# LSquarzoni/SNN_Event-based_Optical_Flow

Hardware: AMD Instinct MI355X
Metric: events/sec (train step) LIFFireNet T=10 128x128 (higher is better)
Workload: dtype fp32; 1 GPU; LIFFireNet train step: T=10 x 1000-event windows, 128x128, batch 8/GPU, base_num_channels 8, EventWarping + Adam; global_batch=8, parallelism=dp1, hip_graph=True, launch_order=wavefront

## Files before the change

include/snnflow.h:

```cpp
#ifndef SNNFLOW_H
#define SNNFLOW_H

#include <stdint.h>

#ifdef __cplusplus
extern "C" {
#endif

#define SNNFLOW_ABI_VERSION 41

#define SNNFLOW_E_ARG (-1)
#define SNNFLOW_E_CHANNELS (-2)

#define SNNFLOW_TILE_H 8
#define SNNFLOW_TILE_W 32

typedef struct snnflow_neuron {
    const float* bn_weight;
    const float* bn_bias;
    float* running_mean;
    float* running_var;
    int64_t* num_batches_tracked;
    const float* beta;
    const float* threshold;
// ... 101 lines not shown
    const uint16_t* wd_ff; const uint16_t* wd_rec;
    float* wslab_ff; float* wslab_rec; const float* s_prev; int wslab_accumulate;
    const float* x; int64_t xs_b, xs_c, xs_h, xs_w;
} snnflow_layer_bwd_args;
int snnflow_layer_bwd(const snnflow_layer_bwd_args* a, void* stream);

#define SNNFLOW_MAX_SLOT_TASKS 4
int snnflow_fwd_slot(const snnflow_conv_fwd_args* conv, int nconv, const snnflow_lif_fwd_args* lif,
                     void* stream);
int snnflow_bwd_slot(const snnflow_layer_bwd_args* layer, int nlayer, const snnflow_lif_bwd_args* lif,
                     void* stream);
int snnflow_slot_supported(int c, int cin0);
#define SNNFLOW_MAX_CHAIN_TASKS 7
int snnflow_bwd_chain(const snnflow_layer_bwd_args* layer, int nlayer, const unsigned char* pair,
                      const snnflow_lif_bwd_args* lif, void* stream);
int snnflow_set_pipe(int fwd_tiles_per_block, int bwd_tiles_per_block);
int snnflow_get_pipe(int which);

#define SNNFLOW_MAX_LAYERS 8

typedef struct snnflow_wgrad_step {
    const float* g_cur;
    const float* y;
    const float* x; int64_t xs_b, xs_c, xs_h, xs_w;
    const float* s_prev;
    const float* stats;
    const float* bnc;
    const uint8_t* x_bits; const uint8_t* s_prev_bits;
} snnflow_wgrad_step;
#define SNNFLOW_MAX_WGRAD_STEPS 32
// ... 516 lines not shown
```

snn_event-based_optical_flow_amd/csrc/lif_layers.hip:

```cpp
#include <cmath>
#include <string>
#include <type_traits>

#include "snnflow_dev.h"
#include "snnflow_tile.h"

#ifndef SNNFLOW_PROBE
#define SNNFLOW_PROBE 0
#endif
#define PROBE_OFF(bit) ((SNNFLOW_PROBE & (bit)) != 0)

#ifndef SNNFLOW_SP32
#define SNNFLOW_SP32 2
#endif
#ifndef SNNFLOW_LATE_D_REC8
#define SNNFLOW_LATE_D_REC8 1
#endif
#ifndef SNNFLOW_LATE_D_FF8
#define SNNFLOW_LATE_D_FF8 1
#endif
#ifndef SNNFLOW_EARLY_G_REC8
#define SNNFLOW_EARLY_G_REC8 1
#endif
#ifndef SNNFLOW_L32_WAVES
// ... 2915 lines not shown
        const float m = beta[c] * mem[i] + x[i];
        const bool s = m >= thr[c];
        spk[i] = s ? 1.0f : 0.0f;
        mout[i] = s ? 0.0f : m;
    }
}

constexpr int kSlotTasks = SNNFLOW_MAX_SLOT_TASKS;

enum SlotKind : int {
    SK_HEAD1, SK_HEAD2, SK_HEAD4, SK_HEAD5,
    SK_PLAIN, SK_PLAIN_REC,
    SK_LIF, SK_LIF_REC,
    SK_TOP, SK_TOP_PRED,
    SK_LIF_P, SK_LIF_REC_P,
    SK_CHAIN
};

struct FwdSlotParams {
    snnflow_conv_fwd_args conv[kSlotTasks];
    snnflow_lif_fwd_args lif;
    int kind[kSlotTasks], blk0[kSlotTasks], nblk[kSlotTasks];
    int ntask;
};
constexpr int kBwdTasks = SNNFLOW_MAX_CHAIN_TASKS, kBwdNodes = kBwdTasks + 1;
struct ByteRange { int off, len; };
constexpr int kNrnA0 = offsetof(snnflow_neuron, running_mean), kNrnA1 = offsetof(snnflow_neuron, beta);
constexpr int kNrnB0 = offsetof(snnflow_neuron, momentum), kNrnB1 = offsetof(snnflow_neuron, bn_train);
constexpr int kBwdOffN = offsetof(snnflow_layer_bwd_args, n), kBwdOffP = offsetof(snnflow_layer_bwd_args, prev);
constexpr int kBwdKeepN = 5;
constexpr ByteRange kBwdKeep[kBwdKeepN] = {
    {0, kBwdOffN + kNrnA0},
    {kBwdOffN + kNrnA1, kNrnB0 - kNrnA1},
    {kBwdOffN + kNrnB1, kBwdOffP + kNrnA0 - (kBwdOffN + kNrnB1)},
    {kBwdOffP + kNrnA1, kNrnB0 - kNrnA1},
    {kBwdOffP + kNrnB1, (int)sizeof(snnflow_layer_bwd_args) - (kBwdOffP + kNrnB1)}};
constexpr int bwd_keep_bytes(int n) { return n == 0 ? 0 : bwd_keep_bytes(n - 1) + kBwdKeep[n - 1].len; }
constexpr bool bwd_keep_aligned(int n) {
    return n == 0 || (kBwdKeep[n - 1].off % 8 == 0 && kBwdKeep[n - 1].len % 8 == 0 && kBwdKeep[n - 1].len > 0 && bwd_keep_aligned(n - 1));
// ... 19 lines not shown
constexpr int cmax(int a, int b) { return a > b ? a : b; }

template <int C>
constexpr bool kSlotAllKinds = C == 8;

constexpr int kFragC8 = 3 * 3 * 256;
constexpr int kPipeRaw = 2 * HN * 16, kPipeSpk = HN * 8 * 2, kPipeFrag = kFragC8 * 2;
template <bool REC>
struct PipeFwdLds {
    static constexpr int RAWY = 0, RAWM = kPipeRaw, SPK = 2 * kPipeRaw, RSPK = SPK + kPipeSpk;
    static constexpr int FF = RSPK + (REC ? kPipeSpk : 0), FR = FF + kPipeFrag;
    static constexpr int BYTES = FR + (REC ? kPipeFrag : 0);
    static constexpr int FLOATS = BYTES / 4;
};

template <int C>
struct SlotLds {
    static constexpr int FWD_ALL = cmax(cmax(ConvFwdLds<1, C, false, false, 2>::FLOATS, ConvFwdLds<5, C, false, false, 2>::FLOATS),
                                        cmax(ConvFwdLds<C, C, false, false, 2>::FLOATS, ConvFwdLds<C, C, false, true, 2>::FLOATS));
    static constexpr int FWD_P = C == 8 ? PipeFwdLds<true>::FLOATS : 0;
    static constexpr int FWD = cmax(cmax(cmax(kSlotAllKinds<C> ? FWD_ALL : 0, kLifQFwdLds<C>), FWD_P),
                                    cmax(cmax(ConvFwdLds<2, C, false, false, 2>::FLOATS, ConvFwdLds<4, C, false, false, 2>::FLOATS),
                                         cmax(ConvFwdLds<C, C, true, false, 2>::FLOATS, ConvFwdLds<C, C, true, true, 2>::FLOATS)));
    static constexpr bool BFG = C >= 16;
    static constexpr int BWD_ALL = cmax(LayerBwdLds<C, C, false, false, 2>::FLOATS, LayerBwdLds<C, C, false, true, 2>::FLOATS);
    static constexpr int BWD = cmax(cmax(cmax(kSlotAllKinds<C> ? BWD_ALL : 0, kLifQBwdLds<C, true>),
                                         cmax(LayerBwdLds<2, C, false, false, 2>::FLOATS, LayerBwdLds<4, C, false, false, 2>::FLOATS)),
                                    cmax(LayerBwdLds<C, C, true, false, 2, BFG>::FLOATS,
                                         LayerBwdLds<C, C, true, true, 2, BFG>::FLOATS));
};

template <typename T>
__device__ inline T kernarg_copy(const __attribute__((address_space(4))) T* p) {
    static_assert(sizeof(T) % 4 == 0, "dword-sized struct");
    T r;
// ... 347 lines not shown
        if ((lane & 15) == 0) {
#pragma unroll
            for (int j = 0; j < 8; ++j) red[wv][lane >> 4][j] = v[j];
        }
        __syncthreads();
        if (tid < 2 * C) {
            const int c = tid & 7, sq = tid >> 3, qd = c >> 2, j = sq * 4 + (c & 3);
            double s = 0.0;
#pragma unroll
            for (int w = 0; w < 8; ++w) s += (double)red[w][qd][j] + (double)red[w][qd + 2][j];
            atomicAdd(acc_shard(a.acc, 2 * C, g.bid) + sq * C + c, s);
        }
    }
}

template <int C>
__global__ __launch_bounds__(NT * 2, C == 8 ? 6 : 1) void k_fwd_slot(FwdSlotParams) {
    typedef const __attribute__((address_space(4))) FwdSlotParams* cptr;
    const cptr pp = (cptr)__builtin_amdgcn_kernarg_segment_ptr();
    Grid g;
    const int k = slot_task(pp, g);
    if (g.bid >= g.nb) return;
    __shared__ __attribute__((aligned(16))) float pool[SlotLds<C>::FWD];
    switch (pp->kind[k]) {
#define FWD_CONV(ALL, KIND, ...)                              \
    case KIND: {                                              \
        if constexpr (ALL || kSlotAllKinds<C>) {              \
            const snnflow_conv_fwd_args a = task_args(&pp->conv[k]);         \
            conv_fwd_body<__VA_ARGS__>(a, g, pool);           \
        }                                                     \
        break;                                                \
    }
        FWD_CONV(false, SK_HEAD1, 1, C, false, false, 2)
        FWD_CONV(true, SK_HEAD2, 2, C, false, false, 2)
        FWD_CONV(true, SK_HEAD4, 4, C, false, false, 2)
        FWD_CONV(false, SK_HEAD5, 5, C, false, false, 2)
        FWD_CONV(false, SK_PLAIN, C, C, false, false, 2)
        FWD_CONV(false, SK_PLAIN_REC, C, C, false, true, 2)
        FWD_CONV(true, SK_LIF, C, C, true, false, 2)
        FWD_CONV(true, SK_LIF_REC, C, C, true, true, 2)
#undef FWD_CONV
        case SK_LIF_P:
        case SK_LIF_REC_P: {
            if constexpr (C == 8) {
                {
                    const snnflow_conv_fwd_args a = task_args(&pp->conv[k]);
                    if (pp->kind[k] == SK_LIF_REC_P) fwd_lif8_pipe<true>(a, g, pool);
                    else fwd_lif8_pipe<false>(a, g, pool);
                }
            }
            break;
        }
        case SK_TOP: {
            if constexpr (kSlotAllKinds<C>) {
                const snnflow_lif_fwd_args a = task_args(&pp->lif);
                lif_fwd_body<C, false, NT * 2>(a, g);
            }
            break;
        }
        case SK_TOP_PRED: {
            const snnflow_lif_fwd_args a = task_args(&pp->lif);
            if constexpr (C >= 16) lif_fwd_q_body<C, true, NT * 2>(a, g, pool);
            else lif_fwd_body<C, true, NT * 2>(a, g);
            break;
// ... 575 lines not shown
        case 4: return layer_bwd_c<4>(*a, s);
        case 8: return layer_bwd_c<8>(*a, s);
        case 16: return layer_bwd_c<16>(*a, s);
        case 32: return layer_bwd_c<32>(*a, s);
        default: SNN_FAIL(SNNFLOW_E_CHANNELS, "layer_bwd: c must be 4, 8, 16 or 32");
    }
}

static bool slot_c(int c) { return c == 8 || c == 16 || c == 32; }

#ifndef SNNFLOW_SLOT_ORDER
#define SNNFLOW_SLOT_ORDER 1
#endif
static int slot_rank(int kind) {
    switch (kind) {
        case SK_LIF_REC_P: case SK_LIF_P: return 0;
        case SK_LIF_REC: case SK_PLAIN_REC: return 0;
        case SK_LIF: case SK_PLAIN: return 1;
        default: return 2;
    }
}

#ifndef SNNFLOW_SLOT_ORDER8
#define SNNFLOW_SLOT_ORDER8 0
#endif
extern "C++" template <typename A>
static void slot_sort(A* args, int* kind, int* nblk, int n, bool reverse = false) {
    if (!SNNFLOW_SLOT_ORDER) return;
    const int sg = reverse ? -1 : 1;
    for (int i = 1; i < n; ++i)
        for (int j = i; j > 0 && sg * slot_rank(kind[j]) < sg * slot_rank(kind[j - 1]); --j) {
// ... 23 lines not shown
    return (nb + 7) / 8 * 8;
}
static bool pipe_fits(int B, int H, int W, int c) { return (int64_t)B * H * W * c * 4 < ((int64_t)1 << 31); }

int snnflow_slot_supported(int c, int cin0) { return slot_c(c) && (cin0 == 2 || cin0 == 4) ? 1 : 0; }

static int slot_ranges(const int* nblk, int n, int* blk0) {
    int b = 0;
    for (int i = 0; i < n; ++i) {
        blk0[i] = b;
        b += (nblk[i] + 7) / 8 * 8;
    }
    return b;
}

int snnflow_fwd_slot(const snnflow_conv_fwd_args* conv, int nconv, const snnflow_lif_fwd_args* lif, void* stream) {
    const int nt = nconv + (lif ? 1 : 0);
    if (nconv < 0 || nt <= 0 || nt > kSlotTasks || (nconv && !conv)) SNN_FAIL(SNNFLOW_E_ARG, "fwd_slot: task count");
    FwdSlotParams p = {};
    const int c = nconv ? conv[0].c : lif->c;
    const int B = nconv ? conv[0].B : lif->B, H = nconv ? conv[0].H : lif->H, W = nconv ? conv[0].W : lif->W;
    if (!slot_c(c)) SNN_FAIL(SNNFLOW_E_CHANNELS, "fwd_slot: c must be 8, 16 or 32");
    for (int i = 0; i < nconv; ++i) {
        const snnflow_conv_fwd_args& a = conv[i];
        if (const int e = conv_fwd_check(&a)) return e;
        if (a.c != c || a.B != B || a.H != H || a.W != W) SNN_FAIL(SNNFLOW_E_ARG, "fwd_slot: tasks of different shapes");
        int kind;
        if (a.lif_in) {
            if (a.cin != c) SNN_FAIL(SNNFLOW_E_CHANNELS, "fwd_slot: lif_in requires cin == c");
            kind = a.wt_rec ? SK_LIF_REC : SK_LIF;
        } else if (a.wt_rec) {
            if (a.cin != c) SNN_FAIL(SNNFLOW_E_CHANNELS, "fwd_slot: recurrent cell requires cin == c");
            kind = SK_PLAIN_REC;
        } else if (a.cin == c) {
            kind = SK_PLAIN;
        } else if (a.cin == 1 || a.cin == 2 || a.cin == 4 || a.cin == 5) {
            kind = a.cin == 1 ? SK_HEAD1 : a.cin == 2 ? SK_HEAD2 : a.cin == 4 ? SK_HEAD4 : SK_HEAD5;
        } else {
            SNN_FAIL(SNNFLOW_E_CHANNELS, "fwd_slot: unsupported cin");
        }
        if (c != 8 && !(kind == SK_HEAD2 || kind == SK_HEAD4 || kind == SK_LIF || kind == SK_LIF_REC))
            SNN_FAIL(SNNFLOW_E_CHANNELS, "fwd_slot: c = 16 / 32 runs the LIFFireNet task kinds only");
        p.conv[i] = a;
        p.nblk[i] = snnflow_conv_blocks(B, H, W);
        if (c == 8 && g_pipe_fwd > 0 && (kind == SK_LIF || kind == SK_LIF_REC) && pipe_fits(B, H, W, c) &&
            !a.prev_spk_bits && !a.s_prev_bits)
            kind = kind == SK_LIF ? SK_LIF_P : SK_LIF_REC_P;
        p.kind[i] = kind;
    }
    const int tpb = g_pipe_fwd;
    for (int i = 0; i < nconv; ++i) {
        if (p.kind[i] != SK_LIF_P && p.kind[i] != SK_LIF_REC_P) continue;
        const int nt = p.nblk[i];
        p.nblk[i] = pipe_blocks(nt, tpb);
        if (p.nblk[i] > (nt + 7) / 8 * 8) p.nblk[i] = (nt + 7) / 8 * 8;
    }
    if (lif) {
        if (const int e = lif_fwd_check(lif)) return e;
        if (lif->c != c || lif->B != B || lif->H != H || lif->W != W)
            SNN_FAIL(SNNFLOW_E_ARG, "fwd_slot: tasks of different shapes");
        if (c != 8 && !lif->pred_w) SNN_FAIL(SNNFLOW_E_CHANNELS, "fwd_slot: c = 16 / 32 top task needs the prediction");
        p.lif = *lif;
        p.kind[nconv] = lif->pred_w ? SK_TOP_PRED : SK_TOP;
        p.nblk[nconv] = slot_top_blocks(c, B, H, W);
    }
    if (c != 8) slot_sort(p.conv, p.kind, p.nblk, nconv);
    else if (SNNFLOW_SLOT_ORDER8) slot_sort(p.conv, p.kind, p.nblk, nconv, SNNFLOW_SLOT_ORDER8 == 2);
    else if (g_pipe_fwd > 0 && g_pipe_order) slot_sort(p.conv, p.kind, p.nblk, nconv, g_pipe_order == 2);
    p.ntask = nt;
    const int nb = slot_ranges(p.nblk, nt, p.blk0);
    const hipStream_t s = (hipStream_t)stream;
    if (c == 8) hipLaunchKernelGGL(k_fwd_slot<8>, dim3(nb), dim3(2 * NT), 0, s, p);
    else if (c == 16) hipLaunchKernelGGL(k_fwd_slot<16>, dim3(nb), dim3(2 * NT), 0, s, p);
    else hipLaunchKernelGGL(k_fwd_slot<32>, dim3(nb), dim3(2 * NT), 0, s, p);
    SNN_CHECK_LAUNCH();
    return 0;
}

int snnflow_eval_slot(const snnflow_eval_fwd_args* tasks, int n, void* stream) {
    if (!tasks || n <= 0 || n > kEvalTasks) SNN_FAIL(SNNFLOW_E_ARG, "eval_slot: task count");
    EvalSlotParams p = {};
    const int B = tasks[0].B, H = tasks[0].H, W = tasks[0].W;
    for (int i = 0; i < n; ++i) {
        const snnflow_eval_fwd_args& a = tasks[i];
        if (a.c != 8) SNN_FAIL(SNNFLOW_E_CHANNELS, "eval_slot: c must be 8");
        if (a.B != B || a.H != H || a.W != W || B <= 0 || H <= 0 || W <= 0)
            SNN_FAIL(SNNFLOW_E_ARG, "eval_slot: tasks of different or empty shapes");
        if (a.n.bn_train) SNN_FAIL(SNNFLOW_E_ARG, "eval_slot: BatchNorm in train mode needs batch statistics (snnflow_fwd_slot)");
        if (!a.state || !a.wt_ff || !a.n.bn_weight || !a.n.bn_bias || !a.n.running_mean || !a.n.running_var ||
            !a.n.beta || !a.n.threshold)
            SNN_FAIL(SNNFLOW_E_ARG, "eval_slot: missing state, weights or neuron parameters");
// ... 337 lines not shown
```

snn_event-based_optical_flow_amd/csrc/snnflow_tile.h:

```cpp
#pragma once

#include <type_traits>

#include "snnflow_dev.h"

#ifndef SNNFLOW_PIN_PF
#define SNNFLOW_PIN_PF 1
#endif

namespace snnflow {


template <int CIN, int NTH = NT>
__device__ void stage_strided(const float* __restrict__ x, int64_t sb, int64_t sc, int64_t sh, int64_t sw,
                              const Tile& tl, int H, int W, float* tile) {
    constexpr int P = Pad<CIN>::v;
    const int tid = threadIdx.x;
    const float* xb = x + (int64_t)tl.b * sb;
    if (sc == 1) {
        for (int e = tid; e < HN * CIN; e += NTH) {
            const int p = e / CIN, ci = e - p * CIN;
            const int r = p / HWD, cc = p - r * HWD;
            const int h = tl.h0 + r - 1, w = tl.w0 + cc - 1;
            tile[p * P + ci] = in_image(h, w, H, W) ? xb[h * sh + w * sw + ci] : 0.0f;
// ... 642 lines not shown
#pragma unroll
                for (int r = 0; r < 4; ++r) out[(row * TW + c0 + g * 4 + r) * PO + n] = v[r];
            }
        }
    }
}

template <int N>
__device__ inline void pin(float (&v)[N]) {
#pragma unroll
    for (int i = 0; i < N; ++i) asm volatile("" : "+v"(v[i]));
}

constexpr int kSumScratch = 8 * 4 * 48;
__device__ inline float* sum_scratch() {
    __shared__ float buf[kSumScratch];
    return buf;
}

template <int NV, int PARTS, typename Dst>
__device__ void block_atomic_sum_parts(const float (&v)[NV], Dst dst) {
    constexpr int WPP = NT / 64, NW = WPP * PARTS;
    if constexpr (NW * 4 * NV > kSumScratch) {
        __shared__ float wred[NW][NV];
        const int lane = threadIdx.x & 63, wv = threadIdx.x >> 6;
#pragma unroll
        for (int j = 0; j < NV; ++j) {
            const float s = wave_total(v[j]);
            if (lane == 0) wred[wv][j] = s;
        }
        __syncthreads();
// ... 165 lines not shown
```

snn_event-based_optical_flow_amd/snnflow/_lib.py:

```python
import ctypes
import os

import torch

_HERE = os.path.dirname(os.path.abspath(__file__))
LIB_PATH = os.environ.get("SNNFLOW_LIB", os.path.join(_HERE, "libsnnflow.so"))

P = ctypes.c_void_p
I32 = ctypes.c_int
I64 = ctypes.c_int64
F32 = ctypes.c_float
F64 = ctypes.c_double

TILE_H, TILE_W = 8, 32
ABI_VERSION = 41
THETA_SCRATCH = 1024 * 32


class Neuron(ctypes.Structure):
    _fields_ = [("bn_weight", P), ("bn_bias", P), ("running_mean", P), ("running_var", P),
                ("num_batches_tracked", P), ("beta", P), ("threshold", P),
                ("momentum", F64), ("eps", F64), ("bn_train", I32), ("zero_reset", I32)]


# ... 330 lines not shown
    "snnflow_iwe_scratch_floats": (I64, [I32, I32, I32, I32, I32, I32]),
    "snnflow_iwe_acc_doubles": (I32, [I32, I32, I32, I32]),
    "snnflow_iwe_corners": (I32, [P, P, I32, I32, F32, I32, I32, F32, I32, P, P, P]),
    "snnflow_iwe_interpolate": (I32, [P, P, P, I64, I32, I32, I32, I32, P, P]),
    "snnflow_iwe_corners_bwd": (I32, [P, P, I32, I32, F32, I32, I32, F32, P, P, P]),
    "snnflow_iwe_interpolate_bwd": (I32, [P, P, I64, I32, I32, I32, I32, P, P, P]),
    "snnflow_lif_export": (I32, [P, P, P, P, I32, I32, I32, P, P, P]),
    "snnflow_lif_theta_subtract": (I32, [P, P, P, I64, I32, P, P, P]),
    "snnflow_clip_grad_norm": (I32, [P, I64, F32, F32, P, P]),
    "snnflow_clip_grad_norm_large": (I32, [P, I64, F32, F32, P, P, P]),
    "snnflow_clip_adam": (I32, [P, P]),
    "snnflow_eval_slot": (I32, [P, I32, P]),
    "snnflow_count_nonzero": (I32, [P, P, I32, P, P]),
    "snnflow_fwd_slot": (I32, [ctypes.POINTER(ConvFwdArgs), I32, ctypes.POINTER(LifFwdArgs), P]),
    "snnflow_bwd_slot": (I32, [ctypes.POINTER(LayerBwdArgs), I32, ctypes.POINTER(LifBwdArgs), P]),
    "snnflow_bwd_chain": (I32, [ctypes.POINTER(LayerBwdArgs), I32, ctypes.POINTER(ctypes.c_ubyte),
                                ctypes.POINTER(LifBwdArgs), P]),
    "snnflow_slot_supported": (I32, [I32, I32]),
    "snnflow_set_pipe": (I32, [I32, I32]),
    "snnflow_get_pipe": (I32, [I32]),
    "snnflow_frag_halfs": (I32, [I32, I32]),
    "snnflow_unet_conv": (I32, [ctypes.POINTER(UNetConvArgs), P]),
    "snnflow_unet_conv_ksplit": (I32, [ctypes.POINTER(UNetConvArgs)]),
    "snnflow_unet_prep_weights": (I32, [P, I32, I32, I32, P, I32, I32, I32, I32, I32, I32, I32, P, P]),
    "snnflow_unet_wgrad": (I32, [ctypes.POINTER(UNetWgradArgs), P]),
    "snnflow_unet_wgrad_partial_floats": (I64, [ctypes.POINTER(UNetWgradArgs)]),
    "snnflow_unet_wgrad_finalize": (I32, [P, I32, P, I32, I32, I32, I32, I32, I32, P, P]),
    "snnflow_unet_lif_bwd": (I32, [ctypes.POINTER(UNetLifBwdArgs), P]),
    "snnflow_unet_lif_bwd_partial_doubles": (I32, [I32, I32, I32]),
    "snnflow_unet_cell_param_grads": (I32, [P, P, P, I32, I32, P, P, P]),
# ... 151 lines not shown
```

snn_event-based_optical_flow_amd/snnflow/engine.py:

```python
import ctypes
import operator
import os

import torch

from . import _lib
from ._lib import check, lib, ptr



def nhwc_state_strides(B, C, H, W):
    return (B * H * W * C, H * W * C, 1, W * C, C)


def empty_state(B, C, H, W, device):
    return torch.empty_strided((2, B, C, H, W), nhwc_state_strides(B, C, H, W), device=device, dtype=torch.float32)


def as_nhwc_state(s):
    two, B, C, H, W = s.shape
    if s.stride() == nhwc_state_strides(B, C, H, W) and s.dtype == torch.float32:
        return s
    out = empty_state(B, C, H, W, s.device)
    out.copy_(s)
# ... 127 lines not shown
        self.L = len(self.cells)
        self.C = self.cells[0].hidden_size
        self.ws = None
        self.prep = PreppedWeights()
        self.bwd_open = False
        self.flat = None
        self.flat_views = None
        self.pending = []
        self.pending_layers = []
        self.slab_live = [False] * self.L
        self.fuse_wgrad = self.C == 8
        fh = os.environ.get("SNNFLOW_FUSE_HEAD")
        self.fuse_head = (self.C >= 16) if fh is None else fh != "0"
        bc = os.environ.get("SNNFLOW_BWD_CHAIN")
        self.bwd_chain = True if bc is None else bc != "0"
        self.spk_bits = os.environ.get("SNNFLOW_SPK_BITS", "1") != "0"
        self.defer_backward = os.environ.get("SNNFLOW_DEFER_BWD", "1") != "0"
        self.keep_seq_states = False
        self.capture_states = False
        self.final_state_out = None
        self.seq_states = None
        self.prep_stale = True
        self.lifs = [c.lif for c in self.cells]
        self.bns = [getattr(c, "batch_norm", c.bn) for c in self.cells]
        self._plist = None
        self._neurons = None
        self._gen = 0

    def __deepcopy__(self, memo):
        import copy
# ... 863 lines not shown
        s = 1 + max((slot[d] for d in deps(n)), default=-1)
        nl = sum(1 for k, _ in n if k < L)
        while s < len(fill) and fill[s] + nl > max_tasks:
            s += 1
        while len(launches) <= s:
            launches.append([])
            fill.append(0)
        slot[n] = s
        fill[s] += nl
        launches[s].append(n)
    for la in launches:
        la.sort(key=lambda n: -n[0][0])
    return launches


def _state_rows(st_all, fin, T):
    rows = [st_all[t] for t in range(st_all.shape[0])]
    return rows + [fin] if fin is not None else rows


class FireNetSequence(torch.autograd.Function):

    @staticmethod
    def forward(ctx, eng, T, *rest):
        L, C = eng.L, eng.C
        xs = list(rest[:T])
        prev = list(rest[T:T + L])
        B, cin0, H, W = xs[0].shape
        dev = xs[0].device
        for x in xs:
# ... 49 lines not shown
        mem_in = [mem0] + [[states[t - 1][l][0] for l in range(L)] for t in range(1, T)]
        s_prev = [sprev0] + [[states[t - 1][l][1] if eng.rec[l] else None for l in range(L)] for t in range(1, T)]
        neurons = eng.neurons()
        train = [bn.training or not bn.track_running_stats for bn in eng.bns]

        fuse = bool(eng.fuse_wgrad)

        bits_on = eng.spk_bits and C in (16, 32) and not fuse
        need_bits = [bits_on and l < L - 1 for l in range(L)]
        bits = (torch.empty(T, L, B * H * W * C // 8, dtype=torch.uint8, device=dev) if any(need_bits)
                else None)
        bptr = [[bits[t, l].data_ptr() if need_bits[l] else None for l in range(L)] for t in range(T)]

        def spk_skip(l, t):
            return t < T - 1 and not eng.keep_seq_states and ((fuse and not eng.rec[l]) or need_bits[l])
        for tasks in wavefront_slots(T, L + 1):
            convs, top = [], None
            for k, t in tasks:
                if k < L:
                    a = _fwd_conv_args(eng, k, B, H, W, cin0, xs[t], ys[t], stats[t], states[t], mem_in[t],
                                       s_prev[t], facc[t], neurons, train, wfwd, wbwd)
                    if k >= 1 and spk_skip(k - 1, t):
                        a.state_spk_skip = 1
                    if k >= 1 and need_bits[k - 1]:
                        a.prev_spk_bits = bptr[t][k - 1]
                    if eng.rec[k] and t >= 1 and need_bits[k]:
                        a.s_prev_bits, a.s_prev = bptr[t - 1][k], None
                    convs.append(a)
                else:
                    top = _fwd_top_args(eng, B, H, W, ys[t], stats[t], states[t], mem_in[t], facc[t], neurons,
                                        flows[t])
                    if spk_skip(L - 1, t):
                        top.state_spk_skip = 1
            arr = (_lib.ConvFwdArgs * max(len(convs), 1))(*convs)
            _lib.call("fwd_slot", lib.snnflow_fwd_slot, arr, len(convs), ctypes.byref(top) if top is not None else None,
                      s)
        _lib.timer_close()

        if eng.capture_states:
            eng.seq_debug = (ys, stats, facc)
        for l in range(L):
            cells[l].lif.mem = states[T - 1][l][0].detach()
        eng.seq_states = [[st.detach() for st in sts] for sts in states] if eng.keep_seq_states else None

        ctx.eng = eng
        ctx.T = T
        ctx.fuse = fuse
        ctx.bptr = bptr
        ctx.bits = bits
        ctx.root = root
        ctx.ext = ext
# ... 246 lines not shown
```

Measured before the change: 68.46 million events/s.

## Chain recurrent layer and following feed-forward layer in one forward pipelined task

Adds a forward chained task (SK_FCHAIN) that fuses a recurrent layer at step t with the next feed-forward layer at step t-1 inside one block. The recurrent layer's spikes are handed over in LDS instead of being reloaded, and the tile loads for the two halves are interleaved. The Python scheduler builds a new wavefront that groups these pairs, which should cut the number of forward launches and the global traffic. In exchange the argument struct and LDS footprint grow, and the dependency graph becomes more intricate.

```diff
diff --git a/include/snnflow.h b/include/snnflow.h
--- a/include/snnflow.h
+++ b/include/snnflow.h
@@ -139,6 +139,8 @@
 #define SNNFLOW_MAX_CHAIN_TASKS 7
 int snnflow_bwd_chain(const snnflow_layer_bwd_args* layer, int nlayer, const unsigned char* pair,
                       const snnflow_lif_bwd_args* lif, void* stream);
+int snnflow_fwd_chain(const snnflow_conv_fwd_args* conv, int nconv, const unsigned char* pair,
+                      const snnflow_lif_fwd_args* lif, void* stream);
 int snnflow_set_pipe(int fwd_tiles_per_block, int bwd_tiles_per_block);
 int snnflow_get_pipe(int which);
 
diff --git a/snn_event-based_optical_flow_amd/csrc/lif_layers.hip b/snn_event-based_optical_flow_amd/csrc/lif_layers.hip
--- a/snn_event-based_optical_flow_amd/csrc/lif_layers.hip
+++ b/snn_event-based_optical_flow_amd/csrc/lif_layers.hip
@@ -2953,15 +2953,18 @@
     SK_LIF, SK_LIF_REC,
     SK_TOP, SK_TOP_PRED,
     SK_LIF_P, SK_LIF_REC_P,
-    SK_CHAIN
+    SK_CHAIN,
+    SK_FCHAIN
 };
 
+constexpr int kFwdTasks = SNNFLOW_MAX_CHAIN_TASKS, kFwdNodes = kFwdTasks + 1;
 struct FwdSlotParams {
-    snnflow_conv_fwd_args conv[kSlotTasks];
+    snnflow_conv_fwd_args conv[kFwdTasks];
     snnflow_lif_fwd_args lif;
-    int kind[kSlotTasks], blk0[kSlotTasks], nblk[kSlotTasks];
+    int kind[kFwdNodes], blk0[kFwdNodes], nblk[kFwdNodes], second[kFwdNodes];
     int ntask;
 };
+static_assert(sizeof(FwdSlotParams) + 256 <= 4096, "kernel arguments: 4 KB with the hidden ones");
 constexpr int kBwdTasks = SNNFLOW_MAX_CHAIN_TASKS, kBwdNodes = kBwdTasks + 1;
 struct ByteRange { int off, len; };
 constexpr int kNrnA0 = offsetof(snnflow_neuron, running_mean), kNrnA1 = offsetof(snnflow_neuron, beta);
@@ -3011,11 +3014,12 @@
     static constexpr int FLOATS = BYTES / 4;
 };
 
+constexpr int kChainFwdFloats = (2 * kPipeRaw + 2 * kPipeSpk + 2 * kPipeFrag) / 4;
 template <int C>
 struct SlotLds {
     static constexpr int FWD_ALL = cmax(cmax(ConvFwdLds<1, C, false, false, 2>::FLOATS, ConvFwdLds<5, C, false, false, 2>::FLOATS),
                                         cmax(ConvFwdLds<C, C, false, false, 2>::FLOATS, ConvFwdLds<C, C, false, true, 2>::FLOATS));
-    static constexpr int FWD_P = C == 8 ? PipeFwdLds<true>::FLOATS : 0;
+    static constexpr int FWD_P = C == 8 ? cmax(PipeFwdLds<true>::FLOATS, kChainFwdFloats) : 0;
     static constexpr int FWD = cmax(cmax(cmax(kSlotAllKinds<C> ? FWD_ALL : 0, kLifQFwdLds<C>), FWD_P),
                                     cmax(cmax(ConvFwdLds<2, C, false, false, 2>::FLOATS, ConvFwdLds<4, C, false, false, 2>::FLOATS),
                                          cmax(ConvFwdLds<C, C, true, false, 2>::FLOATS, ConvFwdLds<C, C, true, true, 2>::FLOATS)));
@@ -3393,12 +3397,257 @@
     }
 }
 
+struct ChainFwdLds {
+    static constexpr int RAWY = 0, RAWM = kPipeRaw, SPK = 2 * kPipeRaw, RSPK = SPK + kPipeSpk;
+    static constexpr int FA = RSPK + kPipeSpk, FB = FA + kPipeFrag;
+    static constexpr int BYTES = FB + kPipeFrag;
+    static constexpr int FLOATS = BYTES / 4;
+    static constexpr int X_FR = 0, X_COEF = kPipeFrag, X_SUMS = X_COEF + 2 * 8 * 16, X_BYTES = X_SUMS + 16 * 8;
+};
+static_assert(ChainFwdLds::BYTES + kPipeFrag == 46464 && ChainFwdLds::FLOATS == kChainFwdFloats, "chained forward pair: LDS budget");
+static_assert(ChainFwdLds::X_BYTES <= kSumScratch * 4 && sizeof(LifCoef) == 16 && ChainFwdLds::X_SUMS % 8 == 0,
+              "chained forward pair: fragments, coefficients and sums in the block-sum scratch");
+
+__device__ inline void chain_issue(const __amdgpu_buffer_rsrc_t rs_y, const __amdgpu_buffer_rsrc_t rs_m, bool has_mem,
+                                   char* lds, const Tile& t, int H, int W, int wv, int lane) {
+    constexpr int C = 8;
+    using L = ChainFwdLds;
+    const int base = ((t.b * H + t.h0 - 1) * W + (t.w0 - 1)) * (C * 4);
+#pragma unroll
+    for (int j = 0; j < 3; ++j) {
+        const int k = wv + 8 * j;
+        if (k >= 22) break;
+        const bool mem = k >= 11;
+        if (mem && !has_mem) continue;
+        const int kk = mem ? k - 11 : k, ee = kk * 64 + lane, p = ee >> 1, r = p / HWD, cc = p - r * HWD;
+        const bool ok = in_image(t.h0 + r - 1, t.w0 + cc - 1, H, W);
+        const uint32_t off = ok ? (uint32_t)(base + (r * W + cc) * (C * 4) + (ee & 1) * 16) : 0x80000000u;
+        if (ee < 2 * HN)
+            __builtin_amdgcn_raw_ptr_buffer_load_lds(mem ? rs_m : rs_y, (lds_void*)(lds + (mem ? L::RAWM : L::RAWY) + kk * 1024),
+                                                     16, off, 0, 0, 0);
+    }
+}
+
+struct ChainHalf {
+    __amdgpu_buffer_rsrc_t rs_y, rs_m;
+    float4* st4;
+    float* y;
+    bool has_mem, zr, spk_skip;
+};
+
+__device__ inline void chain_lif(const ChainHalf& a, int B, int H, int W, const LifCoef* coef, const char* lds, __bf16* spk,
+                                 const Tile& tl, int tid) {
+    constexpr int C = 8, NTB = 2 * NT, R = Halo4<C, NTB>::R;
+    using L = ChainFwdLds;
+    const int qt = tid & 1;
+    const bool has_mem = a.has_mem, zr = a.zr, spk_skip = a.spk_skip;
+    const int64_t plane4 = (int64_t)B * H * W * 2;
+    float4* st4 = a.st4;
+    const LifCoef kc[4] = {coef[4 * qt], coef[4 * qt + 1], coef[4 * qt + 2], coef[4 * qt + 3]};
+#pragma unroll
+    for (int i = 0; i < R; ++i) {
+        const int e = tid + i * NTB;
+        if (e < 2 * HN) {
+            const int p = e >> 1, r = p / HWD, cc = p - r * HWD;
+            const int h = tl.h0 + r - 1, w = tl.w0 + cc - 1;
+            const float4 yv = *reinterpret_cast<const float4*>(lds + L::RAWY + e * 16);
+            const float4 mv = has_mem ? *reinterpret_cast<const float4*>(lds + L::RAWM + e * 16) : make_float4(0.f, 0.f, 0.f, 0.f);
+            float4 sv = make_float4(0.f, 0.f, 0.f, 0.f);
+            if (in_image(h, w, H, W)) {
+                const Lif4 o = zr ? lif_step4(yv, mv, kc, true) : lif_step4(yv, mv, kc, false);
+                sv = o.s;
+                if (r >= 1 && r <= TH && cc >= 1 && cc <= TW) {
+                    const int64_t q = (((int64_t)tl.b * H + h) * W + w) * 2 + qt;
+                    st_state4(st4, q, o.mout);
+                    if (!spk_skip) st_state4(st4, plane4 + q, o.s);
+                }
+            }
+            typedef __bf16 bf16x4 __attribute__((ext_vector_type(4)));
+            *reinterpret_cast<bf16x4*>(spk + p * 8 + 4 * qt) = bf16x4{(__bf16)sv.x, (__bf16)sv.y, (__bf16)sv.z, (__bf16)sv.w};
+        }
+    }
+}
+
+__device__ inline f32x4 chain_conv(bool rec, const char* ff, const char* fr, const __bf16* spk, const __bf16* rspk, int wv,
+                                   int lane) {
+    const int jj = lane & 15, gg = lane >> 4;
+    const bf16x8* fff = reinterpret_cast<const bf16x8*>(ff) + gg * 8 + (jj & 7);
+    const bf16x8* ffr = reinterpret_cast<const bf16x8*>(fr) + gg * 8 + (jj & 7);
+    f32x4 af[2] = {{0.f, 0.f, 0.f, 0.f}, {0.f, 0.f, 0.f, 0.f}}, ar[2] = {{0.f, 0.f, 0.f, 0.f}, {0.f, 0.f, 0.f, 0.f}};
+#pragma unroll
+    for (int ch = 0; ch < 3; ++ch) {
+        const int tap = 4 * ch + gg, ky = tap / 3, kx = tap - 3 * ky;
+        const bf16x8 fh = fff[ch * 96], fm = fff[ch * 96 + 32], fl = fff[ch * 96 + 64];
+#pragma unroll
+        for (int mt = 0; mt < 2; ++mt) {
+            const int off = ((wv + ky) * HWD + mt * 16 + jj + kx) * 8;
+            bf16x8 b = {};
+            if (tap < 9) b = *reinterpret_cast<const bf16x8*>(spk + off);
+            af[mt] = __builtin_amdgcn_mfma_f32_16x16x32_bf16(fl, b, af[mt], 0, 0, 0);
+            af[mt] = __builtin_amdgcn_mfma_f32_16x16x32_bf16(fm, b, af[mt], 0, 0, 0);
+            af[mt] = __builtin_amdgcn_mfma_f32_16x16x32_bf16(fh, b, af[mt], 0, 0, 0);
+        }
+        if (rec) {
+            const bf16x8 rh = ffr[ch * 96], rm = ffr[ch * 96 + 32], rl = ffr[ch * 96 + 64];
+#pragma unroll
+            for (int mt = 0; mt < 2; ++mt) {
+                const int off = ((wv + ky) * HWD + mt * 16 + jj + kx) * 8;
+                bf16x8 b = {};
+                if (tap < 9) b = *reinterpret_cast<const bf16x8*>(rspk + off);
+                ar[mt] = __builtin_amdgcn_mfma_f32_16x16x32_bf16(rl, b, ar[mt], 0, 0, 0);
+                ar[mt] = __builtin_amdgcn_mfma_f32_16x16x32_bf16(rm, b, ar[mt], 0, 0, 0);
+                ar[mt] = __builtin_amdgcn_mfma_f32_16x16x32_bf16(rh, b, ar[mt], 0, 0, 0);
+            }
+        }
+    }
+    f32x4 yv;
+#pragma unroll
+    for (int r = 0; r < 4; ++r) {
+        const float y0 = rec ? af[0][r] + ar[0][r] : af[0][r];
+        const float y1 = rec ? af[1][r] + ar[1][r] : af[1][r];
+        const auto sw = __builtin_amdgcn_permlane32_swap(__builtin_bit_cast(unsigned, y0), __builtin_bit_cast(unsigned, y1),
+                                                         false, false);
+        yv[r] = __builtin_bit_cast(float, sw[0]);
+    }
+    return yv;
+}
+
+__device__ inline void chain_batch_sums(double* acc, const Grid& g, const float (&bs)[4], const float (&bq)[4]) {
+    constexpr int C = 8;
+    const int tid = threadIdx.x, lane = tid & 63, wv = tid >> 6;
+    float v[8] = {bs[0], bs[1], bs[2], bs[3], bq[0], bq[1], bq[2], bq[3]};
+#pragma unroll
+    for (int j = 0; j < 8; ++j) v[j] += dppf<0xB1>(v[j]);
+#pragma unroll
+    for (int j = 0; j < 8; ++j) v[j] += dppf<0x4E>(v[j]);
+#pragma unroll
+    for (int j = 0; j < 8; ++j) v[j] += dppf<0x141>(v[j]);
+#pragma unroll
+    for (int j = 0; j < 8; ++j) v[j] += dppf<0x140>(v[j]);
+    float(*red)[4][8] = reinterpret_cast<float(*)[4][8]>(sum_scratch());
+    if ((lane & 15) == 0) {
+#pragma unroll
+        for (int j = 0; j < 8; ++j) red[wv][lane >> 4][j] = v[j];
+    }
+    __syncthreads();
+    if (acc && tid < 2 * C) {
+        const int c = tid & 7, sq = tid >> 3, qd = c >> 2, j = sq * 4 + (c & 3);
+        double s = 0.0;
+#pragma unroll
+        for (int w = 0; w < 8; ++w) s += (double)red[w][qd][j] + (double)red[w][qd + 2][j];
+        atomicAdd(acc_shard(acc, 2 * C, g.bid) + sq * C + c, s);
+    }
+}
+
+typedef const __attribute__((address_space(4))) snnflow_conv_fwd_args* conv_karg;
+__device__ void fwd_chain8_pipe(const conv_karg pa, const conv_karg pb, const Grid g, float* pool) {
+    constexpr int C = 8;
+    using L = ChainFwdLds;
+    char* const lds = reinterpret_cast<char*>(pool);
+    char* const xlds = reinterpret_cast<char*>(sum_scratch());
+    LifCoef(*coef)[C] = reinterpret_cast<LifCoef(*)[C]>(xlds + L::X_COEF);
+    double* const sums = reinterpret_cast<double*>(xlds + L::X_SUMS);
+    const int lane0 = threadIdx.x & 63;
+    const int wv = __builtin_amdgcn_readfirstlane((int)threadIdx.x >> 6);
+    const int B = pa->B, H = pa->H, W = pa->W, ntiles = B * tiles_per_image(H, W);
+    int v_cur = g.bid < ntiles ? g.bid : -1;
+    if (v_cur < 0) return;
+    const bool lead = g.bid == 0;
+    const uint32_t nbytes = (uint32_t)B * H * W * C * 4;
+    Tile tl = block_tile(H, W, Grid{v_cur, ntiles});
+
+    const bool train_a = pa->prev.bn_train != 0, train_b = pb->prev.bn_train != 0;
+    AccGather<2 * C> gat_a, gat_b;
+    if (train_a) acc_gather_load<2 * C>(as_global_ptr(pa->prev_acc), 2 * C, gat_a);
+    if (train_b) acc_gather_load<2 * C>(as_global_ptr(pb->prev_acc), 2 * C, gat_b);
+    ChainHalf ha, hb;
+    auto prologue = [&](const snnflow_conv_fwd_args& t, const AccGather<2 * C>& gat, LifCoef* cf, ChainHalf& hf, char* frag,
+                        bool first) {
+        const NeuronRegs nr = load_neuron(t.prev, C, lead);
+        FragC8 fz, fzr;
+        fz.load(t.wt_ff_t);
+        if (!first) fzr.load(t.wt_rec_t);
+        hf.has_mem = t.prev_mem != nullptr;
+        hf.zr = t.prev.zero_reset != 0;
+        hf.spk_skip = t.state_spk_skip != 0;
+        hf.st4 = reinterpret_cast<float4*>(t.prev_state);
+        hf.y = t.y;
+        hf.rs_y = __builtin_amdgcn_make_buffer_rsrc(const_cast<float*>(t.prev_y), (short)0, (int)nbytes, 0x00020000);
+        hf.rs_m = __builtin_amdgcn_make_buffer_rsrc(const_cast<float*>(hf.has_mem ? t.prev_mem : t.prev_y), (short)0, (int)nbytes,
+                                                    0x00020000);
+        if (first) chain_issue(hf.rs_y, hf.rs_m, hf.has_mem, lds, tl, H, W, wv, lane0);
+        if (t.prev.bn_train) acc_gather_reduce<2 * C>(gat, sums);
+        lif_prologue(t.prev, nr, sums, C, (double)B * H * W, t.prev_stats, cf, nullptr, lead);
+        fz.store(reinterpret_cast<__bf16*>(frag));
+        if (!first) fzr.store(reinterpret_cast<__bf16*>(xlds + L::X_FR));
+        zero_consumed(t.zero0, t.zero1, t.zero_n, g);
+    };
+    {
+        const snnflow_conv_fwd_args a = task_args(pa);
+        prologue(a, gat_a, coef[0], ha, lds + L::FA, true);
+    }
+    {
+        const snnflow_conv_fwd_args b = task_args(pb);
+        prologue(b, gat_b, coef[1], hb, lds + L::FB, false);
+    }
+
+    float sa[4] = {0.f, 0.f, 0.f, 0.f}, qa[4] = {0.f, 0.f, 0.f, 0.f};
+    float sb[4] = {0.f, 0.f, 0.f, 0.f}, qb[4] = {0.f, 0.f, 0.f, 0.f};
+    __bf16* const spk = reinterpret_cast<__bf16*>(lds + L::SPK);
+    __bf16* const rspk = reinterpret_cast<__bf16*>(lds + L::RSPK);
+
+    Tile cur = tl;
+    for (int second = 0; v_cur >= 0; second ^= 1) {
+        const ChainHalf hf = second ? hb : ha;
+        vm_wait<0>();
+        __syncthreads();
+        chain_lif(hf, B, H, W, coef[second], lds, second ? spk : rspk, cur, opaque_int(threadIdx.x));
+        __syncthreads();
+        int v_nxt = v_cur;
+        if (second) {
+            v_nxt = v_cur + g.nb < ntiles ? v_cur + g.nb : -1;
+            if (v_nxt >= 0) tl = block_tile(H, W, Grid{v_nxt, ntiles});
+        }
+        if (v_nxt >= 0) {
+            const ChainHalf hn = second ? ha : hb;
+            chain_issue(hn.rs_y, hn.rs_m, hn.has_mem, lds, tl, H, W, wv, opaque_int(threadIdx.x) & 63);
+        }
+        const int lane = opaque_int(threadIdx.x) & 63;
+        const f32x4 yv = chain_conv(second != 0, lds + (second ? L::FB : L::FA), xlds + L::X_FR, second ? spk : rspk, rspk, wv, lane);
+        const int qd = (lane >> 4) & 1, h = cur.h0 + wv, w = cur.w0 + (lane >> 5) * 16 + (lane & 15);
+        if (h < H && w < W) {
+            *reinterpret_cast<float4*>(hf.y + (((int64_t)cur.b * H + h) * W + w) * C + 4 * qd) =
+                make_float4(yv[0], yv[1], yv[2], yv[3]);
+            if (second) {
+#pragma unroll
+                for (int r = 0; r < 4; ++r) {
+                    sb[r] += yv[r];
+                    qb[r] += yv[r] * yv[r];
+                }
+            } else {
+#pragma unroll
+                for (int r = 0; r < 4; ++r) {
+                    sa[r] += yv[r];
+                    qa[r] += yv[r] * yv[r];
+                }
+            }
+        }
+        v_cur = v_nxt;
+        cur = tl;
+    }
+
+    __syncthreads();
+    chain_batch_sums(as_global_ptr(pa->acc), g, sa, qa);
+    __syncthreads();
+    chain_batch_sums(as_global_ptr(pb->acc), g, sb, qb);
+}
+
 template <int C>
 __global__ __launch_bounds__(NT * 2, C == 8 ? 6 : 1) void k_fwd_slot(FwdSlotParams) {
     typedef const __attribute__((address_space(4))) FwdSlotParams* cptr;
     const cptr pp = (cptr)__builtin_amdgcn_kernarg_segment_ptr();
     Grid g;
-    const int k = slot_task(pp, g);
+    const int k = slot_task<kFwdNodes>(pp, g);
     if (g.bid >= g.nb) return;
     __shared__ __attribute__((aligned(16))) float pool[SlotLds<C>::FWD];
     switch (pp->kind[k]) {
@@ -3427,6 +3676,12 @@
                     if (pp->kind[k] == SK_LIF_REC_P) fwd_lif8_pipe<true>(a, g, pool);
                     else fwd_lif8_pipe<false>(a, g, pool);
                 }
+            }
+            break;
+        }
+        case SK_FCHAIN: {
+            if constexpr (C == 8) {
+                fwd_chain8_pipe(&pp->conv[k], &pp->conv[pp->second[k]], g, pool);
             }
             break;
         }
@@ -4032,7 +4287,7 @@
 #endif
 static int slot_rank(int kind) {
     switch (kind) {
-        case SK_LIF_REC_P: case SK_LIF_P: return 0;
+        case SK_LIF_REC_P: case SK_LIF_P: case SK_FCHAIN: return 0;
         case SK_LIF_REC: case SK_PLAIN_REC: return 0;
         case SK_LIF: case SK_PLAIN: return 1;
         default: return 2;
@@ -4086,10 +4341,17 @@
     return b;
 }
 
-int snnflow_fwd_slot(const snnflow_conv_fwd_args* conv, int nconv, const snnflow_lif_fwd_args* lif, void* stream) {
-    const int nt = nconv + (lif ? 1 : 0);
-    if (nconv < 0 || nt <= 0 || nt > kSlotTasks || (nconv && !conv)) SNN_FAIL(SNNFLOW_E_ARG, "fwd_slot: task count");
+static int g_fchain_order = env_int("SNNFLOW_FCHAIN_ORDER", 1);
+
+static bool pipe_task(const snnflow_conv_fwd_args& a) {
+    return a.c == 8 && a.cin == 8 && a.lif_in && g_pipe_fwd > 0 && pipe_fits(a.B, a.H, a.W, a.c) && !a.prev_spk_bits &&
+           !a.s_prev_bits;
+}
+
+static int fwd_launch(const snnflow_conv_fwd_args* conv, int nconv, const unsigned char* pair,
+                      const snnflow_lif_fwd_args* lif, void* stream) {
     FwdSlotParams p = {};
+    int taskkind[kFwdTasks], taskblk[kFwdTasks], first[kFwdNodes];
     const int c = nconv ? conv[0].c : lif->c;
     const int B = nconv ? conv[0].B : lif->B, H = nconv ? conv[0].H : lif->H, W = nconv ? conv[0].W : lif->W;
     if (!slot_c(c)) SNN_FAIL(SNNFLOW_E_CHANNELS, "fwd_slot: c must be 8, 16 or 32");
@@ -4113,19 +4375,25 @@
         }
         if (c != 8 && !(kind == SK_HEAD2 || kind == SK_HEAD4 || kind == SK_LIF || kind == SK_LIF_REC))
             SNN_FAIL(SNNFLOW_E_CHANNELS, "fwd_slot: c = 16 / 32 runs the LIFFireNet task kinds only");
-        p.conv[i] = a;
-        p.nblk[i] = snnflow_conv_blocks(B, H, W);
-        if (c == 8 && g_pipe_fwd > 0 && (kind == SK_LIF || kind == SK_LIF_REC) && pipe_fits(B, H, W, c) &&
-            !a.prev_spk_bits && !a.s_prev_bits)
-            kind = kind == SK_LIF ? SK_LIF_P : SK_LIF_REC_P;
-        p.kind[i] = kind;
+        taskblk[i] = snnflow_conv_blocks(B, H, W);
+        if ((kind == SK_LIF || kind == SK_LIF_REC) && pipe_task(a)) kind = kind == SK_LIF ? SK_LIF_P : SK_LIF_REC_P;
+        taskkind[i] = kind;
     }
     const int tpb = g_pipe_fwd;
     for (int i = 0; i < nconv; ++i) {
-        if (p.kind[i] != SK_LIF_P && p.kind[i] != SK_LIF_REC_P) continue;
-        const int nt = p.nblk[i];
-        p.nblk[i] = pipe_blocks(nt, tpb);
-        if (p.nblk[i] > (nt + 7) / 8 * 8) p.nblk[i] = (nt + 7) / 8 * 8;
+        if (taskkind[i] != SK_LIF_P && taskkind[i] != SK_LIF_REC_P) continue;
+        const int nt = taskblk[i];
+        taskblk[i] = pipe_blocks(nt, tpb);
+        if (taskblk[i] > (nt + 7) / 8 * 8) taskblk[i] = (nt + 7) / 8 * 8;
+    }
+    int nn = 0;
+    for (int i = 0; i < nconv; ++i) {
+        const bool ch = pair && pair[i];
+        first[nn] = i;
+        p.kind[nn] = ch ? SK_FCHAIN : taskkind[i];
+        p.nblk[nn] = taskblk[i];
+        ++nn;
+        if (ch) ++i;
     }
     if (lif) {
         if (const int e = lif_fwd_check(lif)) return e;
@@ -4133,20 +4401,69 @@
             SNN_FAIL(SNNFLOW_E_ARG, "fwd_slot: tasks of different shapes");
         if (c != 8 && !lif->pred_w) SNN_FAIL(SNNFLOW_E_CHANNELS, "fwd_slot: c = 16 / 32 top task needs the prediction");
         p.lif = *lif;
-        p.kind[nconv] = lif->pred_w ? SK_TOP_PRED : SK_TOP;
-        p.nblk[nconv] = slot_top_blocks(c, B, H, W);
-    }
-    if (c != 8) slot_sort(p.conv, p.kind, p.nblk, nconv);
-    else if (SNNFLOW_SLOT_ORDER8) slot_sort(p.conv, p.kind, p.nblk, nconv, SNNFLOW_SLOT_ORDER8 == 2);
-    else if (g_pipe_fwd > 0 && g_pipe_order) slot_sort(p.conv, p.kind, p.nblk, nconv, g_pipe_order == 2);
-    p.ntask = nt;
-    const int nb = slot_ranges(p.nblk, nt, p.blk0);
+        p.kind[nn] = lif->pred_w ? SK_TOP_PRED : SK_TOP;
+        p.nblk[nn] = slot_top_blocks(c, B, H, W);
+    }
+    if (c != 8) slot_sort(first, p.kind, p.nblk, nn);
+    else if (SNNFLOW_SLOT_ORDER8) slot_sort(first, p.kind, p.nblk, nn, SNNFLOW_SLOT_ORDER8 == 2);
+    else if (g_pipe_fwd > 0 && g_pipe_order) slot_sort(first, p.kind, p.nblk, nn, g_pipe_order == 2);
+    if (c == 8 && pair && g_fchain_order) {
+        const bool last = g_fchain_order == 2;
+        for (int i = 1; i < nn; ++i)
+            for (int j = i; j > 0 && (p.kind[j] == SK_FCHAIN) != last && (p.kind[j - 1] == SK_FCHAIN) == last; --j) {
+                const int tf = first[j]; first[j] = first[j - 1]; first[j - 1] = tf;
+                const int tk = p.kind[j]; p.kind[j] = p.kind[j - 1]; p.kind[j - 1] = tk;
+                const int tn = p.nblk[j]; p.nblk[j] = p.nblk[j - 1]; p.nblk[j - 1] = tn;
+            }
+    }
+    int nsec = nn;
+    for (int k = 0; k < nn; ++k) {
+        p.conv[k] = conv[first[k]];
+        if (p.kind[k] == SK_FCHAIN) {
+            p.second[k] = nsec;
+            p.conv[nsec++] = conv[first[k] + 1];
+        }
+    }
+    p.ntask = nn + (lif ? 1 : 0);
+    const int nb = slot_ranges(p.nblk, p.ntask, p.blk0);
     const hipStream_t s = (hipStream_t)stream;
     if (c == 8) hipLaunchKernelGGL(k_fwd_slot<8>, dim3(nb), dim3(2 * NT), 0, s, p);
     else if (c == 16) hipLaunchKernelGGL(k_fwd_slot<16>, dim3(nb), dim3(2 * NT), 0, s, p);
     else hipLaunchKernelGGL(k_fwd_slot<32>, dim3(nb), dim3(2 * NT), 0, s, p);
     SNN_CHECK_LAUNCH();
     return 0;
+}
+
+int snnflow_fwd_slot(const snnflow_conv_fwd_args* conv, int nconv, const snnflow_lif_fwd_args* lif, void* stream) {
+    const int nt = nconv + (lif ? 1 : 0);
+    if (nconv < 0 || nt <= 0 || nt > kSlotTasks || (nconv && !conv)) SNN_FAIL(SNNFLOW_E_ARG, "fwd_slot: task count");
+    return fwd_launch(conv, nconv, nullptr, lif, stream);
+}
+
+int snnflow_fwd_chain(const snnflow_conv_fwd_args* conv, int nconv, const unsigned char* pair,
+                      const snnflow_lif_fwd_args* lif, void* stream) {
+    if (nconv < 0 || nconv > kFwdTasks || nconv + (lif ? 1 : 0) <= 0 || (nconv && !conv))
+        SNN_FAIL(SNNFLOW_E_ARG, "fwd_chain: task count");
+    for (int i = 0; pair && i < nconv; ++i) {
+        if (!pair[i]) continue;
+        if (i + 1 >= nconv || pair[i + 1]) SNN_FAIL(SNNFLOW_E_ARG, "fwd_chain: a pair is two consecutive tasks");
+        const snnflow_conv_fwd_args& a = conv[i];
+        const snnflow_conv_fwd_args& b = conv[i + 1];
+        if (a.c != 8 || a.cin != 8 || b.c != 8 || b.cin != 8 || !a.lif_in || !b.lif_in)
+            SNN_FAIL(SNNFLOW_E_CHANNELS, "fwd_chain: pairs are c = cin = 8 LIF-fed tasks");
+        if (a.B != b.B || a.H != b.H || a.W != b.W) SNN_FAIL(SNNFLOW_E_ARG, "fwd_chain: pair of different shapes");
+        if (a.wt_rec || !b.wt_rec || !b.wt_rec_t)
+            SNN_FAIL(SNNFLOW_E_ARG, "fwd_chain: a pair is (feed-forward task, recurrent task)");
+        if (!pipe_task(a) || !pipe_task(b))
+            SNN_FAIL(SNNFLOW_E_ARG, "fwd_chain: pairs need the forward tile pipeline (SNNFLOW_PIPE_FWD > 0, no spike bit "
+                                    "planes, tensors under 2^31 bytes)");
+        if (b.s_prev) SNN_FAIL(SNNFLOW_E_ARG, "fwd_chain: the first task's spikes are handed to the second task (s_prev NULL)");
+        if (a.prev_state == b.prev_state || a.prev_y == b.prev_y || a.prev_y == b.y || a.y == b.y || a.y == b.prev_y ||
+            (a.prev_acc && a.prev_acc == b.prev_acc))
+            SNN_FAIL(SNNFLOW_E_ARG, "fwd_chain: the first task's layer l-1 is the second task's own layer one step earlier");
+        ++i;
+    }
+    return fwd_launch(conv, nconv, pair, lif, stream);
 }
 
 int snnflow_eval_slot(const snnflow_eval_fwd_args* tasks, int n, void* stream) {
diff --git a/snn_event-based_optical_flow_amd/csrc/snnflow_tile.h b/snn_event-based_optical_flow_amd/csrc/snnflow_tile.h
--- a/snn_event-based_optical_flow_amd/csrc/snnflow_tile.h
+++ b/snn_event-based_optical_flow_amd/csrc/snnflow_tile.h
@@ -680,7 +680,7 @@
 
 constexpr int kSumScratch = 8 * 4 * 48;
 __device__ inline float* sum_scratch() {
-    __shared__ float buf[kSumScratch];
+    __shared__ __attribute__((aligned(16))) float buf[kSumScratch];
     return buf;
 }
 
diff --git a/snn_event-based_optical_flow_amd/snnflow/_lib.py b/snn_event-based_optical_flow_amd/snnflow/_lib.py
--- a/snn_event-based_optical_flow_amd/snnflow/_lib.py
+++ b/snn_event-based_optical_flow_amd/snnflow/_lib.py
@@ -368,6 +368,8 @@
     "snnflow_count_nonzero": (I32, [P, P, I32, P, P]),
     "snnflow_fwd_slot": (I32, [ctypes.POINTER(ConvFwdArgs), I32, ctypes.POINTER(LifFwdArgs), P]),
     "snnflow_bwd_slot": (I32, [ctypes.POINTER(LayerBwdArgs), I32, ctypes.POINTER(LifBwdArgs), P]),
+    "snnflow_fwd_chain": (I32, [ctypes.POINTER(ConvFwdArgs), I32, ctypes.POINTER(ctypes.c_ubyte),
+                                ctypes.POINTER(LifFwdArgs), P]),
     "snnflow_bwd_chain": (I32, [ctypes.POINTER(LayerBwdArgs), I32, ctypes.POINTER(ctypes.c_ubyte),
                                 ctypes.POINTER(LifBwdArgs), P]),
     "snnflow_slot_supported": (I32, [I32, I32]),
diff --git a/snn_event-based_optical_flow_amd/snnflow/engine.py b/snn_event-based_optical_flow_amd/snnflow/engine.py
--- a/snn_event-based_optical_flow_amd/snnflow/engine.py
+++ b/snn_event-based_optical_flow_amd/snnflow/engine.py
@@ -165,6 +165,8 @@
         self.fuse_head = (self.C >= 16) if fh is None else fh != "0"
         bc = os.environ.get("SNNFLOW_BWD_CHAIN")
         self.bwd_chain = True if bc is None else bc != "0"
+        fc = os.environ.get("SNNFLOW_FWD_CHAIN")
+        self.fwd_chain = True if fc is None else fc != "0"
         self.spk_bits = os.environ.get("SNNFLOW_SPK_BITS", "1") != "0"
         self.defer_backward = os.environ.get("SNNFLOW_DEFER_BWD", "1") != "0"
         self.keep_seq_states = False
@@ -1058,6 +1060,59 @@
     return launches
 
 
+def chained_fwd_slots(T, rec, chain=(), max_tasks=_lib.MAX_CHAIN_TASKS):
+    L = len(rec)
+    chain = set(chain)
+    if not all(1 <= r < L - 1 and rec[r] and not rec[r + 1] for r in chain):
+        raise ValueError("chained_fwd_slots: a chained layer is recurrent, LIF-fed and followed by a feed-forward "
+                         "layer below the top")
+    node_of = {}
+    for k in range(L + 1):
+        for t in range(T):
+            if k in chain and t >= 1:
+                node = ((k + 1, t - 1), (k, t))
+            elif k - 1 in chain and t <= T - 2:
+                node = ((k, t), (k - 1, t + 1))
+            else:
+                node = ((k, t),)
+            node_of[(k, t)] = node
+
+    def deps(node):
+        out = set()
+        for k, t in node:
+            if k >= 1:
+                out.add((k - 1, t))
+            if t >= 1:
+                out.add((k, t - 1))
+                if k < L and rec[k]:
+                    out.add((k + 1, t - 1))
+        return {node_of[d] for d in out if d not in node}
+
+    level = {}
+
+    def lvl(node):
+        if node not in level:
+            level[node] = 1 + max((lvl(d) for d in deps(node)), default=-1)
+        return level[node]
+
+    nodes = sorted(set(node_of.values()), key=lambda n: (lvl(n), min(k for k, _ in n), n[0][1]))
+    slot, fill, launches = {}, [], []
+    for n in nodes:
+        s = 1 + max((slot[d] for d in deps(n)), default=-1)
+        nl = sum(1 for k, _ in n if k < L)
+        while s < len(fill) and fill[s] + nl > max_tasks:
+            s += 1
+        while len(launches) <= s:
+            launches.append([])
+            fill.append(0)
+        slot[n] = s
+        fill[s] += nl
+        launches[s].append(n)
+    for la in launches:
+        la.sort(key=lambda n: min(k for k, _ in n))
+    return launches
+
+
 def _state_rows(st_all, fin, T):
     rows = [st_all[t] for t in range(st_all.shape[0])]
     return rows + [fin] if fin is not None else rows
@@ -1137,12 +1192,23 @@
 
         def spk_skip(l, t):
             return t < T - 1 and not eng.keep_seq_states and ((fuse and not eng.rec[l]) or need_bits[l])
-        for tasks in wavefront_slots(T, L + 1):
-            convs, top = [], None
-            for k, t in tasks:
+        chained = (bool(eng.fwd_chain) and C == 8 and L <= _lib.MAX_CHAIN_TASKS and not bits_on
+                   and lib.snnflow_get_pipe(0) > 0 and B * H * W * C * 4 < 2 ** 31)
+        if chained:
+            launches = [[(k, t, len(node) == 2 and i == 1) for node in la for i, (k, t) in enumerate(node)]
+                        for la in chained_fwd_slots(T, eng.rec, chainable_layers(eng.rec))]
+        else:
+            launches = [[(k, t, False) for k, t in tasks] for tasks in wavefront_slots(T, L + 1)]
+        for launch in launches:
+            convs, pairs, top = [], [], None
+            for k, t, second_half in launch:
                 if k < L:
                     a = _fwd_conv_args(eng, k, B, H, W, cin0, xs[t], ys[t], stats[t], states[t], mem_in[t],
                                        s_prev[t], facc[t], neurons, train, wfwd, wbwd)
+                    if second_half:
+                        a.s_prev = None
+                        pairs[-1] = 1
+                    pairs.append(0)
                     if k >= 1 and spk_skip(k - 1, t):
                         a.state_spk_skip = 1
                     if k >= 1 and need_bits[k - 1]:
@@ -1156,8 +1222,13 @@
                     if spk_skip(L - 1, t):
                         top.state_spk_skip = 1
             arr = (_lib.ConvFwdArgs * max(len(convs), 1))(*convs)
-            _lib.call("fwd_slot", lib.snnflow_fwd_slot, arr, len(convs), ctypes.byref(top) if top is not None else None,
-                      s)
+            if chained:
+                _lib.call("fwd_slot", lib.snnflow_fwd_chain, arr, len(convs),
+                          (ctypes.c_ubyte * max(len(pairs), 1))(*pairs),
+                          ctypes.byref(top) if top is not None else None, s)
+            else:
+                _lib.call("fwd_slot", lib.snnflow_fwd_slot, arr, len(convs),
+                          ctypes.byref(top) if top is not None else None, s)
         _lib.timer_close()
 
         if eng.capture_states:
```

Measured after the change: 70.42 million events/s (median of 6 runs). 2.9% higher.
